# Rongjiehuang/FastDiff

Measured on AMD Instinct MI355X. Metric: real-time factor (audio-sec/wall-sec), N=4 reverse steps, 80x864 mel, higher is better.
Workload: dtype f32 results; 2-piece fp16 operands (22 bit) on fp16 MFMA, fp32 accumulate; GEMM as Winograd F(2,3); exact-fp32 twin; 1 GPU; BASELINE configs[1]: LJSpeech shape, batch=8 x 80x864 mel per GPU, N=4, HIP kernels + hipGraph sampler; batch_per_gpu=8, frames=864, reverse_steps=4, graph=True, weights=random init seed 1234 (no checkpoint offline), world_size=1, gpus_visible=1, oversubscribed=False

## Files before the change

### fastdiff_amd/csrc/fd_api.cpp

```cpp
#include <math.h>
#include <stddef.h>
#include <stdio.h>
#include <stdlib.h>
#include <string.h>

#include <algorithm>

#include "fd_kernels.h"
#include "fd_host.h"

std::string g_create_error;

static inline int gx_rows_host(int T) { return std::max(fdk_fast::gx_rows(T), fdk_fast::gw_pairs(T) * (fdk_fast::GW_ROWB / fdk_fast::GX_ROWB)); }

bool fd_prof_stamps(const fdk::Launch &L, const char *name, hipEvent_t *e0, hipEvent_t *e1)
{
    fd_context *c = L.ctx;
    if (c->profile != 1 || L.capturing) return false;
    hipEvent_t ev[2];
    for (int i = 0; i < 2; ++i) {
        if (!c->event_pool.empty()) { ev[i] = c->event_pool.back(); c->event_pool.pop_back(); }
        else if (hipEventCreate(&ev[i]) != hipSuccess) return false;
    }
    ProfEntry pe;
// ... 743 lines not shown
    } else {
        if ((rc = enqueue_steps(h, B, T, N, mode, stream)) != FD_OK) return rc;
        if ((rc = copy_out()) != FD_OK) return rc;
    }
    h->last_B = B; h->last_T = T;
    return fd_mark_tail(h, stream);
}

int fd_sample(fd_handle h, const float *mel, int B, int T, const int *lens, const fd_step *table, int N, int ddim,
              const float *x_T, const float *z, uint64_t seed, float *out, float *seq_out, void *stream_)
{
    std::vector<unsigned long long> ids;
    std::vector<long long> offs;
    if (h) { ids.swap(h->noise_ids); offs.swap(h->noise_offs); }
    int rc = check_common(h, B, T, "fd_sample");
    if (rc != FD_OK) return rc;
    if ((rc = fd_follow_stream(h, (hipStream_t)stream_)) != FD_OK) return rc;
    if (h->gen) {
        if (!mel || !table || !out) FD_FAIL(h, FD_ERR_INVALID, "fd_sample: null pointer");
        if (N <= 0 || N > 1024) FD_FAIL(h, FD_ERR_INVALID, "fd_sample: N=%d outside 1..1024", N);
        if (!ids.empty() && (int)ids.size() != B) FD_FAIL(h, FD_ERR_INVALID, "fd_sample: fd_set_noise_streams gave %d stream ids but B=%d", (int)ids.size(), B);
        for (int b = 0; lens && b < B; ++b)
            if (lens[b] < 1 || lens[b] > T) FD_FAIL(h, FD_ERR_INVALID, "fd_sample: lens[%d] = %d outside [1, T=%d]", b, lens[b], T);
        if ((rc = fdg::sample(h, mel, B, T, lens, table, N, ddim, x_T, z, seed, ids, out, seq_out, (hipStream_t)stream_)) != FD_OK) return rc;
        ++h->ticket_counter;
        h->last_B = B; h->last_T = T;
        return fd_mark_tail(h, (hipStream_t)stream_);
    }
    const bool lazy = h->host_fallback && N >= 1 && N <= 8;
    const int Tp = bucket_frames(h, T);
    if ((rc = check_common(h, B, Tp, "fd_sample")) != FD_OK) return rc;
    const int np = (N >= 1 && N <= 1024) ? hoist_mult(h, B, Tp, N) : 1;
    const bool ws_ok = workspace_fits(h, B, Tp, np);
    fd_context::PendingCall prev;
    if (lazy && ws_ok && h->pending.active && h->pending.lazy) {
        prev = h->pending;
        h->pending.active = false;
    } else if ((rc = fd_settle(h)) != FD_OK) return rc;
    auto finish_prev = [&]() -> int {
        if (!prev.active) return FD_OK;
        unsigned mask = 0;
        const fd_context::PendingCall cur = h->pending;
        h->pending.active = false;
        const int r = resolve_call(h, prev, &mask);
        h->pending = cur;
        prev.active = false;
        return r < 0 ? r : FD_OK;
    };
    if (!mel || !table || !out) { finish_prev(); FD_FAIL(h, FD_ERR_INVALID, "fd_sample: null pointer"); }
    if (N <= 0 || N > 1024) { finish_prev(); FD_FAIL(h, FD_ERR_INVALID, "fd_sample: N=%d outside 1..1024", N); }
    if (!ids.empty() && (int)ids.size() != B) {
        finish_prev();
        FD_FAIL(h, FD_ERR_INVALID, "fd_sample: fd_set_noise_streams gave %d stream ids but B=%d", (int)ids.size(), B);
    }
    if (!offs.empty() && offs.size() != ids.size()) { finish_prev(); FD_FAIL(h, FD_ERR_INVALID, "fd_sample: noise offsets without their stream ids"); }
    for (int b = 0; lens && b < B; ++b)
        if (lens[b] < 1 || lens[b] > T) {
            finish_prev();
            FD_FAIL(h, FD_ERR_INVALID, "fd_sample: lens[%d] = %d outside [1, T=%d]", b, lens[b], T);
        }
    if ((rc = ensure_workspace(h, B, Tp, np)) != FD_OK) { finish_prev(); return rc; }
    fd_context::SampleArgs a;
    a.mel = mel; a.B = B; a.T = T; a.N = N; a.ddim = ddim;
    a.has_lens = lens != nullptr;
    if (lens) a.lens.assign(lens, lens + B);
    a.table.assign(table, table + N);
    a.x_T = x_T; a.z = z; a.seed = seed; a.out = out; a.seq_out = seq_out; a.stream = (hipStream_t)stream_;
    a.ids.swap(ids);
    a.offs.swap(offs);
    const long long ticket = ++h->ticket_counter;
    h->n_pieces = h->n_pieces_redone = h->n_pieces_fp32 = 0;
    h->call_fp32_mask = 0;
    rc = sample_core(h, a, 0u, ticket);
    const int rc_prev = finish_prev();
    h->last_B = B; h->last_T = Tp;
    if (rc != FD_OK || rc_prev != FD_OK) return rc != FD_OK ? rc : rc_prev;
    if (!h->defer_check) return fd_settle(h);
    return FD_OK;
}

int64_t fd_sample_ticket(fd_handle h) { return h ? (int64_t)h->ticket_counter : FD_ERR_INVALID; }

static int ticket_redone(fd_handle h, long long ticket)
{
    for (long long t : h->redone_ring)
        if (t == ticket && t != 0) return 1;
    return 0;
}

int fd_sample_settle(fd_handle h, int64_t ticket)
{
    if (!h) return FD_ERR_INVALID;
    if (ticket <= 0 || ticket > h->ticket_counter) FD_FAIL(h, FD_ERR_INVALID, "fd_sample_settle: unknown ticket %lld", (long long)ticket);
    if (h->pending.active && h->pending.ticket <= ticket) {
        FD_HIP(h, hipSetDevice(h->device));
        unsigned mask = 0;
        const int r = resolve_pending(h, &mask);
        if (r < 0) return r;
    }
    return ticket_redone(h, ticket);
}

int fd_sample_check(fd_handle h)
{
    if (!h) return FD_ERR_INVALID;
    if (!h->pending.active) return 0;
    FD_HIP(h, hipSetDevice(h->device));
    unsigned mask = 0;
    return resolve_pending(h, &mask);
}

int fd_set_noise_streams(fd_handle h, const uint64_t *stream_ids, int B)
{
    if (!h || B < 0 || (B > 0 && !stream_ids)) return FD_ERR_INVALID;
    h->noise_ids.assign(stream_ids, stream_ids + B);
    h->noise_offs.clear();
    return FD_OK;
}

int fd_set_option(fd_handle h, const char *key, const char *value)
{
    if (!h || !key || !value) return FD_ERR_INVALID;
    {
        const int rcs = fd_settle(h);
        if (rcs != FD_OK) return rcs;
    }
    const std::string k(key), v(value);
    static const char *stage_names[ST_COUNT] = {"embed", "first", "dblock", "kp_front", "kp_gemm", "convt", "lvc", "final"};
    auto parse_mode = [&](bool &dst) -> int {
        if (v == "fast") dst = true;
        else if (v == "naive") dst = false;
        else FD_FAIL(h, FD_ERR_INVALID, "fd_set_option: %s expects fast|naive, got '%s'", key, value);
        return FD_OK;
    };
    if (k == "kernels") {
        bool m = true;
        int rc = parse_mode(m);
        if (rc != FD_OK) return rc;
        for (int i = 0; i < ST_COUNT; ++i) h->mode.fast[i] = m;
        return FD_OK;
    }
    if (k.compare(0, 8, "kernels.") == 0) {
        for (int i = 0; i < ST_COUNT; ++i)
            if (k.substr(8) == stage_names[i]) return parse_mode(h->mode.fast[i]);
        FD_FAIL(h, FD_ERR_INVALID, "fd_set_option: unknown stage '%s'", key);
    }
    static const struct { const char *key, *a, *b; void (*set)(fd_context *, bool); } choices[] = {
        {"gemm", "f16x2", "fp32", [](fd_context *c, bool a) { c->mode.gemm_f16 = a; }},
        {"gemm_form", "winograd", "direct", [](fd_context *c, bool a) { c->mode.gemm_wino = a; }},
        {"gemm_tile", "16", "32", [](fd_context *c, bool a) { c->mode.gemm_tile16 = a; }},
        {"lvc", "f16x2", "fp32", [](fd_context *c, bool a) { c->mode.lvc_f16 = a; }},
        {"conv", "f16x2", "fp32", [](fd_context *c, bool a) { c->mode.conv_f16 = a; }},
        {"lvc_h8", "mfma", "valu", [](fd_context *c, bool a) { c->mode.lvc_h8_mfma = a; }},
        {"fallback", "graph", "host", [](fd_context *c, bool a) { c->host_fallback = !a; }},
        {"lvc_dx", "gather", "copy", [](fd_context *c, bool a) { c->lvc_dx_gather = a; }},
        {"mel", "pwg", "tacotron", [](fd_context *c, bool a) { c->mel_variant = a ? MEL_PWG : MEL_TACOTRON; }},
    };
    for (const auto &ch : choices) {
        if (k != ch.key) continue;
        if (v != ch.a && v != ch.b) FD_FAIL(h, FD_ERR_INVALID, "fd_set_option: %s expects %s|%s, got '%s'", key, ch.a, ch.b, value);
        ch.set(h, v == ch.a);
        return FD_OK;
    }
    const bool on = (v == "1" || v == "true" || v == "on");
    if (k == "fuse_final") { h->mode.fuse_final = on; return FD_OK; }
    if (k == "fuse_up") { h->mode.fuse_up = on; return FD_OK; }
    if (k == "fuse_advance") { h->mode.fuse_advance = on; return FD_OK; }
    if (k == "embed_cache") { h->embed_cache = on; return FD_OK; }
    if (k == "hoist") {
        if (v == "auto") h->hoist_mode = 1;
        else if (v == "on") h->hoist_mode = 2;
        else if (v == "off") h->hoist_mode = 0;
        else FD_FAIL(h, FD_ERR_INVALID, "fd_set_option: hoist expects auto|on|off, got '%s'", value);
        return FD_OK;
    }
    if (k == "graph") { h->use_graph = on; return FD_OK; }
    if (k == "defer_check") { h->defer_check = on; return FD_OK; }
    if (k == "t_bucket" || k == "graph_cache") {
        char *end = nullptr;
        const long n = strtol(value, &end, 10);
        if (end == value || *end != 0 || n < 0 || n > 65536 || (k == "graph_cache" && n < 1))
            FD_FAIL(h, FD_ERR_INVALID, "fd_set_option: %s expects an integer (t_bucket: frames, 0 = exact T; graph_cache: graphs kept, >= 1), got '%s'", key, value);
        if (k == "t_bucket") h->t_bucket = (int)n;
        else h->max_graphs = (int)n;
        return FD_OK;
    }
    if (k == "profile") { h->profile = (v == "events") ? 2 : (on ? 1 : 0); return FD_OK; }
    if (k == "taps") { h->mode.keep_taps = on; return FD_OK; }
    FD_FAIL(h, FD_ERR_INVALID, "fd_set_option: unknown option '%s'", key);
}

}
```

### fastdiff_amd/csrc/fd_internal.h

```cpp
#pragma once
#include <hip/hip_runtime.h>
#include <hip/hip_ext.h>
#include <stdint.h>
#include <string.h>
#include <map>
#include <string>
#include <vector>

#include "../../include/fastdiff_hip.h"
#include "../../include/fastdiff_hip_ext.h"
#include "../../include/fastdiff_hip_train.h"
#include "fd_loudness.h"
#include "fd_trim.h"
#include "fd_stoi.h"
#include "fd_pitch.h"
#include "fd_spectral.h"
#include "fd_gl.h"
#include "fd_nnls.h"
#include "fd_bins.h"
#include "fd_mcd.h"

namespace fd {
constexpr int C = 32;
constexpr int COND = 80;
constexpr int HID = 64;
constexpr int NBLK = 3;
constexpr int LAYERS = 4;
constexpr int HOPT = 256;
constexpr int E_IN = 128, E_MID = 512, E_OUT = 512;
constexpr int KLAYER = 2 * C * C * 3;
constexpr int KW = KLAYER * LAYERS;
constexpr int KB = 2 * C * LAYERS;
constexpr int KREC = KW + KB;
__host__ __device__ constexpr int ratio(int n) { return n == 2 ? 4 : 8; }
__host__ __device__ constexpr int hop(int n) { return n == 0 ? 8 : (n == 1 ? 64 : 256); }
__host__ __device__ constexpr int down_factor(int d) { return d == 0 ? 4 : 8; }

__host__ __device__ inline int kernel_row(int out) { return (out & 15) + 16 * (out >> 5); }
__host__ __device__ inline int kernel_tile(int out) { return (out & 31) >> 4; }
__host__ __device__ inline int kernel_index(int layer, int in, int out, int tap)
{
    const int kk = tap * C + in, kg = kk >> 4, g = (kk >> 3) & 1, e = kk & 7;
    const int mt = kernel_tile(out), lane = kernel_row(out) + 32 * g;
    return layer * KLAYER + ((mt * 6 + kg) * 64 + lane) * 8 + e;
}
__host__ __device__ inline int bias_index(int layer, int out) { return KW + layer * 64 + kernel_tile(out) * 32 + kernel_row(out); }
}

struct ConvW {
    const float *w = nullptr;
    const float *b = nullptr;
};

struct DevWeights {
    ConvW first, final_;
    struct { ConvW res, conv[3]; } down[fd::NBLK];
    struct { ConvW fc_t, up, kp_in, kp_res[6], kc, bc, convs[fd::LAYERS]; } blk[fd::NBLK];
    const float *fc_t1_T = nullptr, *fc_t1_b = nullptr, *fc_t2_T = nullptr, *fc_t2_b = nullptr;
    const float *fc_t_T[fd::NBLK] = {}, *fc_t_b[fd::NBLK] = {};
    const float *embed_table = nullptr;
    const float *down_pack[fd::NBLK][4] = {};
    const uint16_t *down_h2[fd::NBLK][4] = {};
    bool dblock_f16_ok = false;
    const float *lvc_conv_pack[fd::NBLK][fd::LAYERS] = {};
    const uint16_t *lvc_conv_h2[fd::NBLK][fd::LAYERS] = {};
    const uint16_t *lvc_conv_h16[fd::LAYERS] = {};
    bool lvc_f16_ok = false;
    const float *kp_in_pack[fd::NBLK] = {};
    const float *kp_res_pack[fd::NBLK][6] = {};
    const uint16_t *kp_in_h2[fd::NBLK] = {};
    const uint16_t *kp_res_h2[fd::NBLK][6] = {};
    bool kpf_f16_ok = false;
    const float *gemm_pack[fd::NBLK] = {};
    const float *gemm_bias[fd::NBLK] = {};
    const uint16_t *gemm_h2_pack[fd::NBLK] = {};
    bool gemm_f16_ok = false;
    const uint16_t *gemm_w_pack[fd::NBLK] = {};
    bool gemm_w_ok = false;
    const float *up_pack[fd::NBLK] = {};
    const uint16_t *up_h2[fd::NBLK] = {};
    bool convt_f16_ok = false;
    const float *final_fuse = nullptr;
    const int *kc_perm = nullptr;
    const int *bc_perm = nullptr;
};

struct StepParams {
    fd_step table[1024];
    const float *z;
    float *seq;
    unsigned long long seed;
    int n_steps;
    int ddim;
    int step_idx;
    int l4;
    const unsigned long long *uids;
    int l4_io;
    long long n4_io;
    const long long *offs4;
};

enum Stage { ST_EMBED = 0, ST_FIRST, ST_DBLOCK, ST_KP_FRONT, ST_KP_GEMM, ST_CONVT, ST_LVC, ST_FINAL, ST_COUNT };

struct StepMode {
    bool fast[ST_COUNT] = {true, true, true, true, true, true, true, true};
    bool gemm_f16 = true;
    bool gemm_wino = true;
    bool gemm_tile16 = true;
    bool lvc_f16 = true;
    bool conv_f16 = true;
    bool lvc_h8_mfma = true;
    bool fuse_final = true;
    bool fuse_up = true;
    bool fuse_advance = true;
    bool keep_taps = false;
    unsigned fp32_mask = 0;
    bool inline_fallback = true;
    bool ragged = false;
    int hoist_np = 1;
    bool hoist_chunk = false;

    bool operator==(const StepMode &o) const
    {
        for (int i = 0; i < ST_COUNT; ++i)
            if (fast[i] != o.fast[i]) return false;
        return gemm_f16 == o.gemm_f16 && gemm_wino == o.gemm_wino && gemm_tile16 == o.gemm_tile16 && lvc_f16 == o.lvc_f16 && conv_f16 == o.conv_f16 &&
               lvc_h8_mfma == o.lvc_h8_mfma && fuse_final == o.fuse_final && fuse_up == o.fuse_up && fuse_advance == o.fuse_advance &&
               keep_taps == o.keep_taps && fp32_mask == o.fp32_mask && inline_fallback == o.inline_fallback && ragged == o.ragged &&
               hoist_np == o.hoist_np && hoist_chunk == o.hoist_chunk;
    }
};

struct Workspace {
    int B = 0;
    int64_t frames = 0;
    int64_t rows = 0;
    float *noise = nullptr;
    float *embed_h2 = nullptr;
    float *a[4] = {};
    float *kp_h0 = nullptr, *kp_hA = nullptr, *kp_hB = nullptr;
    float *kpack = nullptr;
    float *h_f16 = nullptr;
    int *lens_dev = nullptr;
    unsigned long long *uid_dev = nullptr;
    long long *off_dev = nullptr;
    float *xsave = nullptr;
    int *range_flag = nullptr;
    float *xA = nullptr, *xB = nullptr;
    float *xtap[fd::NBLK] = {};
    int64_t pframes = 0, prows = 0, plens = 0;
    float *mel_rep = nullptr;
    float *mel = nullptr;
    float *x = nullptr;
    float *eps_acc = nullptr;
    float *steps = nullptr;
    StepParams *params = nullptr;
    size_t bytes = 0;
};

struct ProfEntry { std::string name; hipEvent_t e0, e1; };
struct Scratch { float *p = nullptr; size_t bytes = 0; };

struct MelTables {
    const float *tab = nullptr;
    const int *fb_lo = nullptr, *fb_n = nullptr, *fb_off = nullptr;
    const float *fb_w = nullptr;
};
enum MelVariant { MEL_PWG = 0, MEL_TACOTRON = 1, MEL_VARIANTS = 2 };

struct FoldedParam { std::vector<float> w, b; };
struct WeightImage {
    std::vector<char> bytes;
    std::vector<std::pair<const void **, size_t>> fields;
    template <class T> void add(const T *&dst, const std::vector<T> &v)
    {
        const size_t off = (bytes.size() + 255) & ~(size_t)255;
        bytes.resize(off + v.size() * sizeof(T));
        memcpy(bytes.data() + off, v.data(), v.size() * sizeof(T));
        fields.push_back({reinterpret_cast<const void **>(&dst), off});
    }
};
namespace fdg {
struct Net;
int validate(const fd_config &c, std::string &why);
int create(fd_context *c);
void destroy(fd_context *c);
int hop_total(const fd_context *c);
int pack_weights(fd_context *c, const std::map<std::string, FoldedParam> &f, WeightImage &img);
int forward(fd_context *c, const float *x, const float *mel, const float *steps, int B, int T, const int *lens, float *eps_out, hipStream_t stream);
int sample(fd_context *c, const float *mel, int B, int T, const int *lens, const fd_step *table, int N, int ddim, const float *x_T, const float *z,
           unsigned long long seed, const std::vector<unsigned long long> &ids, float *out, float *seq_out, hipStream_t stream);
}

struct fd_context {
    fd_config cfg;
    fdg::Net *gen = nullptr;
    int device = 0;
    int num_cus = 256;
    std::string err;
    bool committed = false;
    StepMode mode;
    bool use_graph = true;
    int profile = 0;
    std::vector<unsigned long long> noise_ids;
    std::vector<long long> noise_offs;
    bool host_fallback = true;
    std::map<std::string, std::pair<std::vector<int64_t>, std::vector<float>>> raw;
    void *weight_arena = nullptr;
    size_t weight_bytes = 0;
    DevWeights w;
    void *refresh_dev = nullptr;
    size_t refresh_dev_bytes = 0;
    unsigned *refresh_bad = nullptr;
    hipEvent_t refresh_done = nullptr;
    bool refresh_pending = false;
    long long n_refreshes = 0, n_refresh_graph_drops = 0;
    Workspace ws;
    bool lvc_dx_gather = true;
    std::vector<float> embed_t;
    int embed_B = 0;
    bool embed_valid = false;
    bool embed_cache = true;
    MelTables mel[MEL_VARIANTS];
    int mel_variant = MEL_PWG;
    std::vector<float> mel_bank[MEL_VARIANTS];
    bool mel_bank_user[MEL_VARIANTS] = {false, false};
    std::vector<void *> tables;
    struct KeyedTable { std::vector<float> host; const float *dev = nullptr; };
    std::map<std::pair<int, int>, const float *> resample_tabs;
    int last_B = 0, last_T = 0;
    hipStream_t cap_stream = nullptr;
    hipStream_t last_stream = nullptr;
    bool have_last_stream = false;
    hipEvent_t ev_switch = nullptr;
    bool tail_marked = false;
    int hoist_mode = 1;
    struct StepGraph { int B, T, steps; StepMode mode; hipGraph_t graph; hipGraphExec_t exec; unsigned long long last_use; };
    std::vector<StepGraph> graphs;
    unsigned long long graph_clock = 0;
    struct RetiredGraph { hipGraph_t graph; hipGraphExec_t exec; hipEvent_t done; };
    std::vector<RetiredGraph> retired;
    int max_graphs = 64;
    int t_bucket = 32;
    long long n_graph_captures = 0, n_graph_hits = 0, n_graph_evictions = 0;
    bool defer_check = false;
    static constexpr int STAGE_SLOTS = 8;
    struct StageSlot { char *host = nullptr; size_t cap = 0; hipEvent_t done = nullptr; };
    StageSlot stage[STAGE_SLOTS];
    unsigned stage_next = 0;
    struct SampleArgs {
        const float *mel = nullptr;
        int B = 0, T = 0, N = 0, ddim = 0;
        bool has_lens = false;
        std::vector<int> lens;
        std::vector<fd_step> table;
        const float *x_T = nullptr, *z = nullptr;
        unsigned long long seed = 0;
        float *out = nullptr, *seq_out = nullptr;
        hipStream_t stream = nullptr;
        std::vector<unsigned long long> ids;
        std::vector<long long> offs;
    };
    struct PendingCall {
        bool active = false;
        bool lazy = false;
        int slot = 0;
        long long ticket = 0;
        int B = 0, T = 0, N = 0, first = 0, count = 0;
        int T_io = 0;
        float *out = nullptr;
        hipStream_t stream = nullptr;
        StepMode mode;
        SampleArgs args;
    } pending;
    long long ticket_counter = 0;
    long long n_pieces = 0, n_pieces_redone = 0, n_pieces_fp32 = 0, n_calls_redone = 0;
    unsigned call_fp32_mask = 0;
    long long redone_ring[16] = {};
    unsigned redone_next = 0;
    int *flags_host = nullptr;
    hipEvent_t flags_done = nullptr, flags_done2 = nullptr;
// ... 180 lines not shown
```

### fastdiff_amd/csrc/fd_kernels_dblock.hip

```cpp
#include "fd_kernels_common.h"

namespace fdk_fast {

constexpr int DB_LD = 136;
constexpr int DB_STRIDE = 114;

template <int DIL, bool LRELU>
__device__ __forceinline__ void conv96_tile(f32x16 &acc, const float4 (&wa)[12], const float *in, int ld, int col, int hi)
{
    const int o[3] = {opaque(hi * ld + col - DIL), opaque(hi * ld + col), opaque(hi * ld + col + DIL)};
#pragma unroll
    for (int s = 0; s < 48; ++s) {
        const int tap = s >> 4, c2 = (2 * s) & 31;
        float v = in[o[tap] + c2 * ld];
        if (LRELU) v = lrelu(v, 0.2f);
        acc = mfma32(f4c(wa[s >> 2], s & 3), v, acc);
    }
}

template <int F>
__global__ void __launch_bounds__(256, 2) k_dblock(const float *__restrict__ xin, float *__restrict__ out,
                                                   const float *__restrict__ p0, const float *__restrict__ p1,
                                                   const float *__restrict__ p2, const float *__restrict__ pr,
                                                   const float *__restrict__ b0, const float *__restrict__ b1,
                                                   const float *__restrict__ b2, const float *__restrict__ br, int Lin, int Lo,
                                                   const int *__restrict__ run_if, const int *__restrict__ lens, int per_frame)
{
    __shared__ __attribute__((aligned(16))) float xs[fd::C * DB_LD];
    if (run_if && *run_if == 0) return;
    __shared__ __attribute__((aligned(16))) float hA[fd::C * DB_LD];
    __shared__ __attribute__((aligned(16))) float hB[fd::C * DB_LD];
    const int b = blockIdx.y, tid = threadIdx.x, lane = tid & 63, wave = tid >> 6, l31 = lane & 31, hi = lane >> 5;
    const int pbase = blockIdx.x * DB_STRIDE - 7;
    const int Lob = lens ? lens[b] * per_frame : Lo;
    if (blockIdx.x * DB_STRIDE >= Lob) return;
    {
        constexpr int NK = fd::C * DB_LD / 256;
        float v[NK];
#pragma unroll
        for (int k = 0; k < NK; ++k) {
            const int idx = k * 256 + tid, ci = idx / DB_LD, cc = idx - ci * DB_LD, p = pbase + cc - 4;
            v[k] = (cc >= 4 && cc < 132 && p >= 0 && p < Lob) ? xin[((int64_t)b * fd::C + ci) * Lin + (int64_t)p * F] : 0.0f;
        }
#pragma unroll
        for (int k = 0; k < NK; ++k) {
            const int idx = k * 256 + tid;
            xs[idx] = v[k];
            hA[idx] = 0.0f;
            hB[idx] = 0.0f;
        }
    }
    __syncthreads();
    const int c = wave * 32 + l31;
    const int p = pbase + c;
    const bool inside = (p >= 0 && p < Lob);
    float4 wa[12];
    f32x16 acc;
#pragma unroll
    for (int i = 0; i < 12; ++i) wa[i] = reinterpret_cast<const float4 *>(p0)[i * 64 + lane];
#pragma unroll
    for (int r = 0; r < 16; ++r) acc[r] = b0[drow(r, hi)];
    conv96_tile<1, true>(acc, wa, xs, DB_LD, 4 + c, hi);
#pragma unroll
    for (int r = 0; r < 16; ++r) hA[drow(r, hi) * DB_LD + 4 + c] = inside ? acc[r] : 0.0f;
    __syncthreads();
#pragma unroll
    for (int i = 0; i < 12; ++i) wa[i] = reinterpret_cast<const float4 *>(p1)[i * 64 + lane];
#pragma unroll
    for (int r = 0; r < 16; ++r) acc[r] = b1[drow(r, hi)];
    conv96_tile<2, true>(acc, wa, hA, DB_LD, 4 + c, hi);
#pragma unroll
    for (int r = 0; r < 16; ++r) hB[drow(r, hi) * DB_LD + 4 + c] = inside ? acc[r] : 0.0f;
    __syncthreads();
#pragma unroll
    for (int i = 0; i < 12; ++i) wa[i] = reinterpret_cast<const float4 *>(p2)[i * 64 + lane];
#pragma unroll
    for (int r = 0; r < 16; ++r) acc[r] = b2[drow(r, hi)] + br[drow(r, hi)];
    conv96_tile<4, true>(acc, wa, hB, DB_LD, 4 + c, hi);
    {
        float4 wr[4];
#pragma unroll
        for (int i = 0; i < 4; ++i) wr[i] = reinterpret_cast<const float4 *>(pr)[i * 64 + lane];
#pragma unroll
        for (int s = 0; s < 16; ++s) acc = mfma32(f4c(wr[s >> 2], s & 3), xs[(2 * s + hi) * DB_LD + 4 + c], acc);
    }
    if (inside && c >= 7 && c < 7 + DB_STRIDE) {
#pragma unroll
        for (int r = 0; r < 16; ++r) out[((int64_t)b * fd::C + drow(r, hi)) * Lo + p] = acc[r];
    }
}

constexpr int DBH_ROWS = 136;

template <int DIL>
__device__ __forceinline__ void conv96_h2(f32x16 &ah, f32x16 &al, const float4 (&wa)[2][6], const char *img, int c, int hi)
{
    int off[3][2][2];
#pragma unroll
    for (int tap = 0; tap < 3; ++tap)
#pragma unroll
        for (int p = 0; p < 2; ++p)
#pragma unroll
            for (int c2 = 0; c2 < 2; ++c2) off[tap][p][c2] = h2_off(4 + c + (tap - 1) * DIL, p * 4 + c2 * 2 + hi);
#pragma unroll
    for (int kg = 0; kg < 6; ++kg) {
        const float4 b1 = *reinterpret_cast<const float4 *>(img + off[kg >> 1][0][kg & 1]);
        const float4 b2 = *reinterpret_cast<const float4 *>(img + off[kg >> 1][1][kg & 1]);
        ah = mfma_f16(wa[0][kg], b1, ah);
        al = mfma_f16(wa[0][kg], b2, al);
        al = mfma_f16(wa[1][kg], b1, al);
    }
}
__device__ __forceinline__ void store_act_h2(char *img, const f32x16 &ah, const f32x16 &al, int c, int hi, bool inside, float &mx)
{
    const int row = 4 + c;
#pragma unroll
    for (int j = 0; j < 4; ++j) {
        float v[4];
#pragma unroll
        for (int i = 0; i < 4; ++i) {
            v[i] = inside ? lrelu(fmaf(al[4 * j + i], GX_INV_SCALE, ah[4 * j + i]), 0.2f) : 0.0f;
            mx = fmaxf(mx, fabsf(v[i]));
        }
        uint2 ph, pl;
        split2(v[0], v[1], ph.x, pl.x);
        split2(v[2], v[3], ph.y, pl.y);
        *reinterpret_cast<uint2 *>(img + h2_off(row, j) + 8 * hi) = ph;
        *reinterpret_cast<uint2 *>(img + h2_off(row, 4 + j) + 8 * hi) = pl;
    }
}

#ifndef FD_DBLOCK_OCC
#define FD_DBLOCK_OCC 3
#endif
template <int F, bool AUDIO>
__global__ void __launch_bounds__(256, FD_DBLOCK_OCC) k_dblock_h2(const float *__restrict__ xin, float *__restrict__ out,
                                                      const float4 *__restrict__ p0, const float4 *__restrict__ p1,
                                                      const float4 *__restrict__ p2, const float4 *__restrict__ pr,
                                                      const float *__restrict__ b0, const float *__restrict__ b1,
                                                      const float *__restrict__ b2, const float *__restrict__ br, int Lin, int Lo,
                                                      int *__restrict__ range_flag, const int *__restrict__ lens, int per_frame,
                                                      const float *__restrict__ audio, const float *__restrict__ fw,
                                                      const float *__restrict__ fb)
{
    __shared__ __attribute__((aligned(16))) char xl[DBH_ROWS * 128];
    __shared__ __attribute__((aligned(16))) char xr[DBH_ROWS * 128];
    __shared__ __attribute__((aligned(16))) char ha[DBH_ROWS * 128];
    const int b = blockIdx.y, tid = threadIdx.x, lane = tid & 63, wave = tid >> 6, l31 = lane & 31, hi = lane >> 5;
    const int pbase = blockIdx.x * DB_STRIDE - 7;
    const int Lob = lens ? lens[b] * per_frame : Lo;
    if (blockIdx.x * DB_STRIDE >= Lob || skip_after_previous_overflow(range_flag)) return;
    float mx = 0.0f;
    __shared__ float fwl[AUDIO ? 256 : 1];
    if constexpr (AUDIO) {
        fwl[tid] = tid < 224 ? fw[tid] : fb[tid - 224];
        __syncthreads();
    }
    {
        float v[2][8];
#pragma unroll
        for (int k = 0; k < 2; ++k) {
            const int u = k * 256 + tid, cg = u >> 7, cc = u & 127, p = pbase + cc;
            const bool ok = p >= 0 && p < Lob;
            if (AUDIO) {
                const int Lb = Lob * F, t = p * F;
                const float *xa = audio + (int64_t)b * Lin;
                float xv[7];
#pragma unroll
                for (int i = 0; i < 7; ++i) xv[i] = (ok && t - 3 + i >= 0 && t - 3 + i < Lb) ? xa[t - 3 + i] : 0.0f;
                const int o0 = __builtin_amdgcn_readfirstlane(cg) * 8;
#pragma unroll
                for (int c = 0; c < 8; ++c) {
                    float r = fwl[224 + o0 + c];
#pragma unroll
                    for (int i = 0; i < 7; ++i) r += fwl[(o0 + c) * 7 + i] * xv[i];
                    v[k][c] = ok ? r : 0.0f;
                }
            } else {
#pragma unroll
                for (int c = 0; c < 8; ++c) v[k][c] = ok ? xin[((int64_t)b * fd::C + cg * 8 + c) * Lin + (int64_t)p * F] : 0.0f;
            }
        }
        if (tid < 128) {
            const int g = tid >> 4, row = g < 4 ? g : 128 + g, part = tid & 15;
            *reinterpret_cast<uint2 *>(xl + row * 128 + part * 8) = make_uint2(0u, 0u);
            *reinterpret_cast<uint2 *>(xr + row * 128 + part * 8) = make_uint2(0u, 0u);
            *reinterpret_cast<uint2 *>(ha + row * 128 + part * 8) = make_uint2(0u, 0u);
        }
#pragma unroll
        for (int k = 0; k < 2; ++k) {
            const int u = k * 256 + tid, cg = u >> 7, cc = u & 127;
            float a[8];
#pragma unroll
            for (int c = 0; c < 8; ++c) { mx = fmaxf(mx, fabsf(v[k][c])); a[c] = lrelu(v[k][c], 0.2f); }
            float4 ph, pl;
            split8(v[k], ph, pl);
            *reinterpret_cast<float4 *>(xr + h2_off(4 + cc, cg)) = ph;
            *reinterpret_cast<float4 *>(xr + h2_off(4 + cc, 4 + cg)) = pl;
            split8(a, ph, pl);
            *reinterpret_cast<float4 *>(xl + h2_off(4 + cc, cg)) = ph;
            *reinterpret_cast<float4 *>(xl + h2_off(4 + cc, 4 + cg)) = pl;
        }
    }
    __syncthreads();
    const int c = wave * 32 + l31;
    const int p = pbase + c;
    const bool inside = (p >= 0 && p < Lob);
    float4 wa[2][6];
    f32x16 ah, al;
    auto load_w = [&](const float4 *pk) {
#pragma unroll
        for (int q = 0; q < 2; ++q)
#pragma unroll
            for (int kg = 0; kg < 6; ++kg) wa[q][kg] = pk[(q * 6 + kg) * 64 + lane];
    };
    load_w(p0);
#pragma unroll
    for (int r = 0; r < 16; ++r) { ah[r] = b0[drow(r, hi)]; al[r] = 0.0f; }
    conv96_h2<1>(ah, al, wa, xl, c, hi);
    store_act_h2(ha, ah, al, c, hi, inside, mx);
    __syncthreads();
    load_w(p1);
#pragma unroll
    for (int r = 0; r < 16; ++r) { ah[r] = b1[drow(r, hi)]; al[r] = 0.0f; }
    conv96_h2<2>(ah, al, wa, ha, c, hi);
    store_act_h2(xl, ah, al, c, hi, inside, mx);
    __syncthreads();
    load_w(p2);
#pragma unroll
    for (int r = 0; r < 16; ++r) { ah[r] = b2[drow(r, hi)] + br[drow(r, hi)]; al[r] = 0.0f; }
    conv96_h2<4>(ah, al, wa, xl, c, hi);
    {
        float4 wr[2][2];
#pragma unroll
        for (int q = 0; q < 2; ++q)
#pragma unroll
            for (int kg = 0; kg < 2; ++kg) wr[q][kg] = pr[(q * 2 + kg) * 64 + lane];
#pragma unroll
        for (int kg = 0; kg < 2; ++kg) {
            const float4 x1 = *reinterpret_cast<const float4 *>(xr + h2_off(4 + c, kg * 2 + hi));
            const float4 x2 = *reinterpret_cast<const float4 *>(xr + h2_off(4 + c, 4 + kg * 2 + hi));
            ah = mfma_f16(wr[0][kg], x1, ah);
            al = mfma_f16(wr[0][kg], x2, al);
            al = mfma_f16(wr[1][kg], x1, al);
        }
    }
    if (inside && c >= 7 && c < 7 + DB_STRIDE) {
#pragma unroll
        for (int r = 0; r < 16; ++r) out[((int64_t)b * fd::C + drow(r, hi)) * Lo + p] = fmaf(al[r], GX_INV_SCALE, ah[r]);
    }
    if (!(mx < GX_LIMIT)) atomicOr(range_flag, 1);
}

}

namespace fdk {
using namespace fdk_fast;

hipError_t fast_dblock(const Launch &L, int d, int B, int T, const float *audio)
{
    fd_context *c = L.ctx;
    const DevWeights &w = c->w;
    int Lin = T * fd::HOPT;
    for (int i = 0; i < d; ++i) Lin /= fd::down_factor(i);
    const int f = fd::down_factor(d), Lo = Lin / f;
    const dim3 grid((Lo + DB_STRIDE - 1) / DB_STRIDE, B);
    const int *run_if = nullptr;
    const char *n4 = "dblock_f4", *n8 = "dblock_f8";
    const int *lens = L.mode->ragged ? c->ws.lens_dev : nullptr;
    const Pipe pipe = fd_pipe(*L.mode, L.mode->conv_f16 && w.dblock_f16_ok, 13 + d);
    if (pipe != PIPE_F32_ONLY) {
        int *flag = c->ws.range_flag + 13 + d;
        const float4 *q0 = reinterpret_cast<const float4 *>(w.down_h2[d][0]), *q1 = reinterpret_cast<const float4 *>(w.down_h2[d][1]),
                     *q2 = reinterpret_cast<const float4 *>(w.down_h2[d][2]), *q3 = reinterpret_cast<const float4 *>(w.down_h2[d][3]);
        const float *none = nullptr;
        if (f == 4 && d == 0 && audio)
            FD_LAUNCH(L, n4, (k_dblock_h2<4, true>), grid, dim3(256), 0, c->ws.a[d], c->ws.a[d + 1], q0, q1, q2, q3, w.down[d].conv[0].b,
                      w.down[d].conv[1].b, w.down[d].conv[2].b, w.down[d].res.b, Lin, Lo, flag, lens, Lo / T, audio,
                      (const float *)w.first.w, (const float *)w.first.b);
        else if (f == 4)
            FD_LAUNCH(L, n4, (k_dblock_h2<4, false>), grid, dim3(256), 0, c->ws.a[d], c->ws.a[d + 1], q0, q1, q2, q3, w.down[d].conv[0].b,
                      w.down[d].conv[1].b, w.down[d].conv[2].b, w.down[d].res.b, Lin, Lo, flag, lens, Lo / T, none, none, none);
        else
            FD_LAUNCH(L, n8, (k_dblock_h2<8, false>), grid, dim3(256), 0, c->ws.a[d], c->ws.a[d + 1], q0, q1, q2, q3, w.down[d].conv[0].b,
                      w.down[d].conv[1].b, w.down[d].conv[2].b, w.down[d].res.b, Lin, Lo, flag, lens, Lo / T, none, none, none);
        run_if = flag;
        n4 = n8 = "dblock_fp32_fallback";
        if (pipe == PIPE_F16_ONLY) return hipSuccess;
    }
    if (f == 4)
        FD_LAUNCH(L, n4, k_dblock<4>, grid, dim3(256), 0, c->ws.a[d], c->ws.a[d + 1], w.down_pack[d][0], w.down_pack[d][1],
                  w.down_pack[d][2], w.down_pack[d][3], w.down[d].conv[0].b, w.down[d].conv[1].b, w.down[d].conv[2].b,
                  w.down[d].res.b, Lin, Lo, run_if, lens, Lo / T);
    else
        FD_LAUNCH(L, n8, k_dblock<8>, grid, dim3(256), 0, c->ws.a[d], c->ws.a[d + 1], w.down_pack[d][0], w.down_pack[d][1],
                  w.down_pack[d][2], w.down_pack[d][3], w.down[d].conv[0].b, w.down[d].conv[1].b, w.down[d].conv[2].b,
                  w.down[d].res.b, Lin, Lo, run_if, lens, Lo / T);
    return hipSuccess;
}

}
```

Before: 10200 x real-time.

## Add persistent walking form of f16x2 downsampling block kernel with prefetch

Adds a persistent variant of the fp16-pair downsampling block kernel, launched with at most CUs times occupancy workgroups. Each workgroup walks (batch, tile) items in strides and skips tiles past the ragged length. While the last conv of the current tile runs, it prefetches the next tile's inputs into registers and reloads the first-layer weights. Biases and first-layer audio weights are staged in LDS once per workgroup. This targets launch and tail overhead and hides global-load latency, at the cost of more register pressure and a serial walk per workgroup.

Measured after the change: 10260 x real-time (median of 6 runs). Within noise of the previous version (+0.5%).

```diff
diff --git a/fastdiff_amd/csrc/fd_api.cpp b/fastdiff_amd/csrc/fd_api.cpp
--- a/fastdiff_amd/csrc/fd_api.cpp
+++ b/fastdiff_amd/csrc/fd_api.cpp
@@ -919,6 +919,7 @@
         {"lvc", "f16x2", "fp32", [](fd_context *c, bool a) { c->mode.lvc_f16 = a; }},
         {"conv", "f16x2", "fp32", [](fd_context *c, bool a) { c->mode.conv_f16 = a; }},
         {"lvc_h8", "mfma", "valu", [](fd_context *c, bool a) { c->mode.lvc_h8_mfma = a; }},
+        {"dblock_form", "persistent", "tile", [](fd_context *c, bool a) { c->mode.dblock_persistent = a; }},
         {"fallback", "graph", "host", [](fd_context *c, bool a) { c->host_fallback = !a; }},
         {"lvc_dx", "gather", "copy", [](fd_context *c, bool a) { c->lvc_dx_gather = a; }},
         {"mel", "pwg", "tacotron", [](fd_context *c, bool a) { c->mel_variant = a ? MEL_PWG : MEL_TACOTRON; }},
@@ -943,12 +944,13 @@
     }
     if (k == "graph") { h->use_graph = on; return FD_OK; }
     if (k == "defer_check") { h->defer_check = on; return FD_OK; }
-    if (k == "t_bucket" || k == "graph_cache") {
+    if (k == "t_bucket" || k == "graph_cache" || k == "dblock_wgs") {
         char *end = nullptr;
         const long n = strtol(value, &end, 10);
         if (end == value || *end != 0 || n < 0 || n > 65536 || (k == "graph_cache" && n < 1))
-            FD_FAIL(h, FD_ERR_INVALID, "fd_set_option: %s expects an integer (t_bucket: frames, 0 = exact T; graph_cache: graphs kept, >= 1), got '%s'", key, value);
+            FD_FAIL(h, FD_ERR_INVALID, "fd_set_option: %s expects an integer (t_bucket: frames, 0 = exact T; graph_cache: graphs kept, >= 1; dblock_wgs: workgroups, 0 = all resident), got '%s'", key, value);
         if (k == "t_bucket") h->t_bucket = (int)n;
+        else if (k == "dblock_wgs") h->mode.dblock_wgs = (int)n;
         else h->max_graphs = (int)n;
         return FD_OK;
     }
diff --git a/fastdiff_amd/csrc/fd_dblock_walk.h b/fastdiff_amd/csrc/fd_dblock_walk.h
--- /dev/null
+++ b/fastdiff_amd/csrc/fd_dblock_walk.h
@@ -0,0 +1,53 @@
+#pragma once
+
+#if defined(__HIPCC__)
+#define FD_DBW_FN __host__ __device__ __forceinline__
+#else
+#define FD_DBW_FN inline
+#endif
+
+namespace fdk_dbw {
+
+constexpr int COLS = 128;
+constexpr int STRIDE = 114;
+constexpr int HALO = 7;
+
+struct Item {
+    int item;
+    int b, tile;
+    int Lob;
+};
+
+FD_DBW_FN int tiles_of(int Lo) { return (Lo + STRIDE - 1) / STRIDE; }
+
+FD_DBW_FN int workgroups(int n_items, int resident, int cap)
+{
+    int n = n_items < resident ? n_items : resident;
+    if (cap > 0 && cap < n) n = cap;
+    return n < 1 ? 1 : n;
+}
+
+FD_DBW_FN Item live_from(int item, int step, int n_items, int tiles, const int *lens, int per_frame, int Lo)
+{
+    for (; item < n_items; item += step) {
+        const int b = item / tiles, tile = item - b * tiles;
+        const int Lob = lens ? lens[b] * per_frame : Lo;
+        if (tile * STRIDE < Lob) return Item{item, b, tile, Lob};
+    }
+    return Item{-1, 0, 0, 0};
+}
+
+FD_DBW_FN int pbase_of(int tile) { return tile * STRIDE - HALO; }
+
+FD_DBW_FN int pick_column(int pbase, int cc, int Lob)
+{
+    const int p = pbase + cc;
+    return p < 0 ? 0 : (p < Lob ? p : Lob - 1);
+}
+FD_DBW_FN int audio_sample(int pbase, int cc, int i, int F, int Lob)
+{
+    const int t = (pbase + cc) * F - 3 + i, Lb = Lob * F;
+    return t < 0 ? 0 : (t < Lb ? t : Lb - 1);
+}
+
+}
diff --git a/fastdiff_amd/csrc/fd_internal.h b/fastdiff_amd/csrc/fd_internal.h
--- a/fastdiff_amd/csrc/fd_internal.h
+++ b/fastdiff_amd/csrc/fd_internal.h
@@ -113,6 +113,8 @@
     bool fuse_final = true;
     bool fuse_up = true;
     bool fuse_advance = true;
+    bool dblock_persistent = true;
+    int dblock_wgs = 0;
     bool keep_taps = false;
     unsigned fp32_mask = 0;
     bool inline_fallback = true;
@@ -126,7 +128,7 @@
             if (fast[i] != o.fast[i]) return false;
         return gemm_f16 == o.gemm_f16 && gemm_wino == o.gemm_wino && gemm_tile16 == o.gemm_tile16 && lvc_f16 == o.lvc_f16 && conv_f16 == o.conv_f16 &&
                lvc_h8_mfma == o.lvc_h8_mfma && fuse_final == o.fuse_final && fuse_up == o.fuse_up && fuse_advance == o.fuse_advance &&
-               keep_taps == o.keep_taps && fp32_mask == o.fp32_mask && inline_fallback == o.inline_fallback && ragged == o.ragged &&
+               dblock_persistent == o.dblock_persistent && dblock_wgs == o.dblock_wgs && keep_taps == o.keep_taps && fp32_mask == o.fp32_mask && inline_fallback == o.inline_fallback && ragged == o.ragged &&
                hoist_np == o.hoist_np && hoist_chunk == o.hoist_chunk;
     }
 };
diff --git a/fastdiff_amd/csrc/fd_kernels_dblock.hip b/fastdiff_amd/csrc/fd_kernels_dblock.hip
--- a/fastdiff_amd/csrc/fd_kernels_dblock.hip
+++ b/fastdiff_amd/csrc/fd_kernels_dblock.hip
@@ -1,4 +1,7 @@
+#include <type_traits>
+
 #include "fd_kernels_common.h"
+#include "fd_dblock_walk.h"
 
 namespace fdk_fast {
 
@@ -133,19 +136,173 @@
 #ifndef FD_DBLOCK_OCC
 #define FD_DBLOCK_OCC 3
 #endif
+constexpr int DB_WALK_OCC = 3;
+static_assert(DB_STRIDE == fdk_dbw::STRIDE && DBH_ROWS == fdk_dbw::COLS + 8, "fd_dblock_walk.h states the same tiling");
 template <int F, bool AUDIO>
-__global__ void __launch_bounds__(256, FD_DBLOCK_OCC) k_dblock_h2(const float *__restrict__ xin, float *__restrict__ out,
-                                                      const float4 *__restrict__ p0, const float4 *__restrict__ p1,
-                                                      const float4 *__restrict__ p2, const float4 *__restrict__ pr,
-                                                      const float *__restrict__ b0, const float *__restrict__ b1,
-                                                      const float *__restrict__ b2, const float *__restrict__ br, int Lin, int Lo,
-                                                      int *__restrict__ range_flag, const int *__restrict__ lens, int per_frame,
-                                                      const float *__restrict__ audio, const float *__restrict__ fw,
-                                                      const float *__restrict__ fb)
-{
-    __shared__ __attribute__((aligned(16))) char xl[DBH_ROWS * 128];
-    __shared__ __attribute__((aligned(16))) char xr[DBH_ROWS * 128];
-    __shared__ __attribute__((aligned(16))) char ha[DBH_ROWS * 128];
+__device__ __forceinline__ void dblock_h2_walk(char *xl, char *xr, char *ha, const float *__restrict__ xin, float *__restrict__ out,
+                                               const float4 *__restrict__ p0, const float4 *__restrict__ p1,
+                                               const float4 *__restrict__ p2, const float4 *__restrict__ pr,
+                                               const float *__restrict__ b0, const float *__restrict__ b1,
+                                               const float *__restrict__ b2, const float *__restrict__ br, int Lin, int Lo,
+                                               int *__restrict__ range_flag, const int *__restrict__ lens, int per_frame,
+                                               const float *__restrict__ audio, const float *__restrict__ fw,
+                                               const float *__restrict__ fb, int tiles, int n_items)
+{
+    __shared__ float fwl[AUDIO ? 256 : 1];
+    __shared__ __attribute__((aligned(16))) float bl[3 * fd::C];
+    const int tid0 = threadIdx.x;
+    const int n_wg = gridDim.x;
+    if (skip_after_previous_overflow(range_flag)) return;
+    fdk_dbw::Item it = fdk_dbw::live_from(blockIdx.x, n_wg, n_items, tiles, lens, per_frame, Lo);
+    if (it.item < 0) return;
+    constexpr int NX = AUDIO ? 7 : 8;
+    float nx[2][NX];
+    auto request = [&](const fdk_dbw::Item &q, int tid) {
+        const int pbase = fdk_dbw::pbase_of(q.tile);
+#pragma unroll
+        for (int k = 0; k < 2; ++k) {
+            const int u = k * 256 + tid, cg = u >> 7, cc = u & 127;
+            if constexpr (AUDIO) {
+                const float *xa = audio + (int64_t)q.b * Lin;
+#pragma unroll
+                for (int i = 0; i < 7; ++i) nx[k][i] = xa[(unsigned)fdk_dbw::audio_sample(pbase, cc, i, F, q.Lob)];
+            } else {
+                const int64_t at = (int64_t)fdk_dbw::pick_column(pbase, cc, q.Lob) * F;
+#pragma unroll
+                for (int c = 0; c < 8; ++c) nx[k][c] = xin[((int64_t)q.b * fd::C + cg * 8 + c) * Lin + at];
+            }
+        }
+    };
+    float4 wa[2][6], wr[2][2];
+    auto load_w = [&](const float4 *pk, int lane) {
+#pragma unroll
+        for (int q = 0; q < 2; ++q)
+#pragma unroll
+            for (int kg = 0; kg < 6; ++kg) wa[q][kg] = pk[(q * 6 + kg) * 64 + lane];
+    };
+    auto bias = [&](f32x16 &ah, f32x16 &al, int layer, int hi) {
+#pragma unroll
+        for (int r = 0; r < 16; ++r) { ah[r] = bl[layer * fd::C + drow(r, hi)]; al[r] = 0.0f; }
+    };
+    request(it, tid0);
+    load_w(p0, tid0 & 63);
+    if constexpr (AUDIO) fwl[tid0] = tid0 < 224 ? fw[tid0] : fb[tid0 - 224];
+    if (tid0 < 3 * fd::C) {
+        const int ch = tid0 & (fd::C - 1);
+        bl[tid0] = tid0 < fd::C ? b0[ch] : (tid0 < 2 * fd::C ? b1[ch] : b2[ch] + br[ch]);
+    }
+    if (tid0 < 128) {
+        const int g = tid0 >> 4, row = g < 4 ? g : 128 + g, part = tid0 & 15;
+        *reinterpret_cast<uint2 *>(xl + row * 128 + part * 8) = make_uint2(0u, 0u);
+        *reinterpret_cast<uint2 *>(xr + row * 128 + part * 8) = make_uint2(0u, 0u);
+        *reinterpret_cast<uint2 *>(ha + row * 128 + part * 8) = make_uint2(0u, 0u);
+    }
+    __syncthreads();
+    float mx = 0.0f;
+    auto pass = [&](auto more, const fdk_dbw::Item &it, const fdk_dbw::Item &nxt) {
+        constexpr bool MORE = decltype(more)::value;
+        const int tid = opaque(tid0), lane = tid & 63, wave = tid >> 6, l31 = lane & 31, hi = lane >> 5;
+        const int c = wave * 32 + l31;
+        const int pbase = fdk_dbw::pbase_of(it.tile), Lob = it.Lob;
+#pragma unroll
+        for (int k = 0; k < 2; ++k) {
+            const int u = k * 256 + tid, cg = u >> 7, cc = u & 127, p = pbase + cc;
+            const bool ok = p >= 0 && p < Lob;
+            float v[8];
+            if constexpr (AUDIO) {
+                const int Lb = Lob * F, t = p * F;
+                float xv[7];
+#pragma unroll
+                for (int i = 0; i < 7; ++i) xv[i] = (ok && t - 3 + i >= 0 && t - 3 + i < Lb) ? nx[k][i] : 0.0f;
+                const int o0 = __builtin_amdgcn_readfirstlane(cg) * 8;
+#pragma unroll
+                for (int ch = 0; ch < 8; ++ch) {
+                    float r = fwl[224 + o0 + ch];
+#pragma unroll
+                    for (int i = 0; i < 7; ++i) r += fwl[(o0 + ch) * 7 + i] * xv[i];
+                    v[ch] = ok ? r : 0.0f;
+                }
+            } else {
+#pragma unroll
+                for (int ch = 0; ch < 8; ++ch) v[ch] = ok ? nx[k][ch] : 0.0f;
+            }
+            float a[8];
+#pragma unroll
+            for (int ch = 0; ch < 8; ++ch) { mx = fmaxf(mx, fabsf(v[ch])); a[ch] = lrelu(v[ch], 0.2f); }
+            float4 ph, pl;
+            split8(v, ph, pl);
+            *reinterpret_cast<float4 *>(xr + h2_off(4 + cc, cg)) = ph;
+            *reinterpret_cast<float4 *>(xr + h2_off(4 + cc, 4 + cg)) = pl;
+            split8(a, ph, pl);
+            *reinterpret_cast<float4 *>(xl + h2_off(4 + cc, cg)) = ph;
+            *reinterpret_cast<float4 *>(xl + h2_off(4 + cc, 4 + cg)) = pl;
+        }
+        __syncthreads();
+        const int p = pbase + c;
+        const bool inside = (p >= 0 && p < Lob);
+        f32x16 ah, al;
+        bias(ah, al, 0, hi);
+        conv96_h2<1>(ah, al, wa, xl, c, hi);
+        __builtin_amdgcn_sched_barrier(0);
+        load_w(p1, lane);
+        __builtin_amdgcn_sched_barrier(0);
+        store_act_h2(ha, ah, al, c, hi, inside, mx);
+        __syncthreads();
+        bias(ah, al, 1, hi);
+        conv96_h2<2>(ah, al, wa, ha, c, hi);
+        __builtin_amdgcn_sched_barrier(0);
+        load_w(p2, lane);
+        __builtin_amdgcn_sched_barrier(0);
+        store_act_h2(xl, ah, al, c, hi, inside, mx);
+        __syncthreads();
+#pragma unroll
+        for (int q = 0; q < 2; ++q)
+#pragma unroll
+            for (int kg = 0; kg < 2; ++kg) wr[q][kg] = pr[(q * 2 + kg) * 64 + lane];
+        bias(ah, al, 2, hi);
+        conv96_h2<4>(ah, al, wa, xl, c, hi);
+        __builtin_amdgcn_sched_barrier(0);
+        if constexpr (MORE) request(nxt, tid);
+        __builtin_amdgcn_sched_barrier(0);
+#pragma unroll
+        for (int kg = 0; kg < 2; ++kg) {
+            const float4 x1 = *reinterpret_cast<const float4 *>(xr + h2_off(4 + c, kg * 2 + hi));
+            const float4 x2 = *reinterpret_cast<const float4 *>(xr + h2_off(4 + c, 4 + kg * 2 + hi));
+            ah = mfma_f16(wr[0][kg], x1, ah);
+            al = mfma_f16(wr[0][kg], x2, al);
+            al = mfma_f16(wr[1][kg], x1, al);
+        }
+        __builtin_amdgcn_sched_barrier(0);
+        if constexpr (MORE) load_w(p0, lane);
+        __builtin_amdgcn_sched_barrier(0);
+        if (inside && c >= 7 && c < 7 + DB_STRIDE) {
+            float *ob = out + (int64_t)it.b * fd::C * Lo;
+#pragma unroll
+            for (int r = 0; r < 16; ++r) ob[(unsigned)drow(r, hi) * (unsigned)Lo + (unsigned)p] = fmaf(al[r], GX_INV_SCALE, ah[r]);
+        }
+        if constexpr (MORE) __syncthreads();
+    };
+    fdk_dbw::Item nxt = fdk_dbw::live_from(it.item + n_wg, n_wg, n_items, tiles, lens, per_frame, Lo);
+    while (nxt.item >= 0) {
+        const fdk_dbw::Item after = fdk_dbw::live_from(nxt.item + n_wg, n_wg, n_items, tiles, lens, per_frame, Lo);
+        pass(std::true_type(), it, nxt);
+        it = nxt;
+        nxt = after;
+    }
+    pass(std::false_type(), it, nxt);
+    if (!(mx < GX_LIMIT)) atomicOr(range_flag, 1);
+}
+
+template <int F, bool AUDIO>
+__device__ __forceinline__ void dblock_h2_tile(char *xl, char *xr, char *ha, const float *__restrict__ xin, float *__restrict__ out,
+                                               const float4 *__restrict__ p0, const float4 *__restrict__ p1,
+                                               const float4 *__restrict__ p2, const float4 *__restrict__ pr,
+                                               const float *__restrict__ b0, const float *__restrict__ b1,
+                                               const float *__restrict__ b2, const float *__restrict__ br, int Lin, int Lo,
+                                               int *__restrict__ range_flag, const int *__restrict__ lens, int per_frame,
+                                               const float *__restrict__ audio, const float *__restrict__ fw,
+                                               const float *__restrict__ fb)
+{
     const int b = blockIdx.y, tid = threadIdx.x, lane = tid & 63, wave = tid >> 6, l31 = lane & 31, hi = lane >> 5;
     const int pbase = blockIdx.x * DB_STRIDE - 7;
     const int Lob = lens ? lens[b] * per_frame : Lo;
@@ -250,6 +407,26 @@
         for (int r = 0; r < 16; ++r) out[((int64_t)b * fd::C + drow(r, hi)) * Lo + p] = fmaf(al[r], GX_INV_SCALE, ah[r]);
     }
     if (!(mx < GX_LIMIT)) atomicOr(range_flag, 1);
+}
+
+template <int F, bool AUDIO, bool PERSIST>
+__global__ void __launch_bounds__(256, PERSIST ? DB_WALK_OCC : FD_DBLOCK_OCC) k_dblock_h2(const float *__restrict__ xin, float *__restrict__ out,
+                                                      const float4 *__restrict__ p0, const float4 *__restrict__ p1,
+                                                      const float4 *__restrict__ p2, const float4 *__restrict__ pr,
+                                                      const float *__restrict__ b0, const float *__restrict__ b1,
+                                                      const float *__restrict__ b2, const float *__restrict__ br, int Lin, int Lo,
+                                                      int *__restrict__ range_flag, const int *__restrict__ lens, int per_frame,
+                                                      const float *__restrict__ audio, const float *__restrict__ fw,
+                                                      const float *__restrict__ fb, int tiles, int n_items)
+{
+    __shared__ __attribute__((aligned(16))) char xl[DBH_ROWS * 128];
+    __shared__ __attribute__((aligned(16))) char xr[DBH_ROWS * 128];
+    __shared__ __attribute__((aligned(16))) char ha[DBH_ROWS * 128];
+    if constexpr (PERSIST)
+        dblock_h2_walk<F, AUDIO>(xl, xr, ha, xin, out, p0, p1, p2, pr, b0, b1, b2, br, Lin, Lo, range_flag, lens, per_frame, audio, fw, fb,
+                                 tiles, n_items);
+    else
+        dblock_h2_tile<F, AUDIO>(xl, xr, ha, xin, out, p0, p1, p2, pr, b0, b1, b2, br, Lin, Lo, range_flag, lens, per_frame, audio, fw, fb);
 }
 
 }
@@ -274,16 +451,25 @@
         const float4 *q0 = reinterpret_cast<const float4 *>(w.down_h2[d][0]), *q1 = reinterpret_cast<const float4 *>(w.down_h2[d][1]),
                      *q2 = reinterpret_cast<const float4 *>(w.down_h2[d][2]), *q3 = reinterpret_cast<const float4 *>(w.down_h2[d][3]);
         const float *none = nullptr;
-        if (f == 4 && d == 0 && audio)
-            FD_LAUNCH(L, n4, (k_dblock_h2<4, true>), grid, dim3(256), 0, c->ws.a[d], c->ws.a[d + 1], q0, q1, q2, q3, w.down[d].conv[0].b,
-                      w.down[d].conv[1].b, w.down[d].conv[2].b, w.down[d].res.b, Lin, Lo, flag, lens, Lo / T, audio,
-                      (const float *)w.first.w, (const float *)w.first.b);
-        else if (f == 4)
-            FD_LAUNCH(L, n4, (k_dblock_h2<4, false>), grid, dim3(256), 0, c->ws.a[d], c->ws.a[d + 1], q0, q1, q2, q3, w.down[d].conv[0].b,
-                      w.down[d].conv[1].b, w.down[d].conv[2].b, w.down[d].res.b, Lin, Lo, flag, lens, Lo / T, none, none, none);
-        else
-            FD_LAUNCH(L, n8, (k_dblock_h2<8, false>), grid, dim3(256), 0, c->ws.a[d], c->ws.a[d + 1], q0, q1, q2, q3, w.down[d].conv[0].b,
-                      w.down[d].conv[1].b, w.down[d].conv[2].b, w.down[d].res.b, Lin, Lo, flag, lens, Lo / T, none, none, none);
+        const bool first = f == 4 && d == 0 && audio;
+        const float *au = first ? audio : none, *fw = first ? (const float *)w.first.w : none, *fb = first ? (const float *)w.first.b : none;
+        const int tiles = (int)grid.x, n_items = tiles * B;
+        const dim3 walk(fdk_dbw::workgroups(n_items, c->num_cus * DB_WALK_OCC, L.mode->dblock_wgs));
+#define FD_DBLOCK_H2(NAME_, F_, AUDIO_)                                                                                                    \
+    do {                                                                                                                                   \
+        if (L.mode->dblock_persistent && (int64_t)fd::C * Lo < (1ll << 32))        \
+            FD_LAUNCH(L, NAME_, (k_dblock_h2<F_, AUDIO_, true>), walk, dim3(256), 0, c->ws.a[d], c->ws.a[d + 1], q0, q1, q2, q3,          \
+                      w.down[d].conv[0].b, w.down[d].conv[1].b, w.down[d].conv[2].b, w.down[d].res.b, Lin, Lo, flag, lens, Lo / T, au, fw,   \
+                      fb, tiles, n_items);                                                                                                 \
+        else                                                                                                                               \
+            FD_LAUNCH(L, NAME_, (k_dblock_h2<F_, AUDIO_, false>), grid, dim3(256), 0, c->ws.a[d], c->ws.a[d + 1], q0, q1, q2, q3,         \
+                      w.down[d].conv[0].b, w.down[d].conv[1].b, w.down[d].conv[2].b, w.down[d].res.b, Lin, Lo, flag, lens, Lo / T, au, fw,   \
+                      fb, tiles, n_items);                                                                                                 \
+    } while (0)
+        if (first) FD_DBLOCK_H2(n4, 4, true);
+        else if (f == 4) FD_DBLOCK_H2(n4, 4, false);
+        else FD_DBLOCK_H2(n8, 8, false);
+#undef FD_DBLOCK_H2
         run_if = flag;
         n4 = n8 = "dblock_fp32_fallback";
         if (pipe == PIPE_F16_ONLY) return hipSuccess;
```
